# cloneofsimo/paint-with-words-sd

Measured on AMD Instinct MI355X. Metric: 512x512 images/sec (30 steps, CFG) SD1.5+PwW, higher is better.
Workload: dtype bf16

## Files before the change

include/pww_hip_linear.h:

```cpp
#ifndef PWW_HIP_LINEAR_H
#define PWW_HIP_LINEAR_H

#include "pww_hip.h"

#ifdef __cplusplus
extern "C" {
#endif

#define PWW_LINEAR_VERSION 100

int pww_linear_version(void);
const char *pww_linear_last_error(void);

#define PWW_LINEAR_NONE 0
#define PWW_LINEAR_BIAS 1
#define PWW_LINEAR_BIAS_RESIDUAL 2
#define PWW_LINEAR_BIAS_GEGLU 3
typedef struct pww_linear_desc {
    uint32_t size;
    int32_t dtype;
    int32_t M, N, K;
    int32_t epilogue;
    int64_t x_stride, y_stride, r_stride;
    int32_t tile_n, splitk;
} pww_linear_desc_t;
size_t pww_linear_workspace_bytes(const pww_linear_desc_t *desc);
int pww_linear_fwd(const void *x, const void *w, const void *bias, const void *residual, void *y, const pww_linear_desc_t *desc, void *workspace,
                   size_t workspace_bytes, void *stream);

#ifdef __cplusplus
}
#endif

#endif
```

paint-with-words-sd_amd/build.py:

```python
import os
import subprocess
import sys

HERE = os.path.dirname(os.path.abspath(__file__))
REPO = os.path.dirname(HERE)
CSRC = os.path.join(HERE, "csrc")
LIB = os.path.join(HERE, "pww_hip", "libpww_hip.so")
LIB_EXPERIMENTS = os.path.join(HERE, "pww_hip", "libpww_hip_experiments.so")
UNITS = [("pww_api.hip", [], ""), ("pww_attn.hip", [], ""), ("pww_cross.hip", [], ""), ("pww_cross_lean.hip", [], ""), ("pww_reduce.hip", [], ""),
         ("pww_mask.hip", [], ""), ("pww_qproj.hip", [], ""), ("pww_norm.hip", [], ""), ("pww_blocks.hip", [], ""), ("pww_conv.hip", [], ""), ("pww_probs.hip", [], ""),
         ("pww_attn_inst.hip", ["-DPWW_INST_F16"], ".f16"), ("pww_attn_inst.hip", ["-DPWW_INST_BF16"], ".bf16"),
         ("pww_cross_inst.hip", ["-DPWW_INST_F16", "-DPWW_INST_NW=2"], ".f16.nw2"), ("pww_cross_inst.hip", ["-DPWW_INST_F16", "-DPWW_INST_NW=4"], ".f16.nw4"),
         ("pww_cross_inst.hip", ["-DPWW_INST_BF16", "-DPWW_INST_NW=2"], ".bf16.nw2"), ("pww_cross_inst.hip", ["-DPWW_INST_BF16", "-DPWW_INST_NW=4"], ".bf16.nw4")]
EXPERIMENT_UNITS = [("pww_cross_out.hip", [], "")]
_ATTN_HEADERS = ["pww_tile.h", "pww_attn_core.h", "pww_cross_tile.h"]
SIDE_FLAGS = ["-fvisibility=hidden"]
SIDE_LIBS = {
    "long": ("pww_long.hip", _ATTN_HEADERS, "the long-prompt launches"),
    "scope": ("pww_scope.hip", _ATTN_HEADERS, "cross-attention with per-head / per-row score statistics"),
    "linear": ("pww_linear.hip", [], "linear layers with a bias / residual / GEGLU epilogue"),
    "regions": ("pww_regions.hip", [], "region masks and the per-pixel blend of the noise predictions"),
    "lora": ("pww_lora.hip", [], "the per-row low-rank update of unmerged LoRA adapters"),
}
SOURCES = sorted({u[0] for u in UNITS + EXPERIMENT_UNITS})
HEADERS = ["pww_common.h", "pww_tile.h", "pww_attn_core.h", "pww_attn_kernel.h", "pww_cross_tile.h", "pww_cross_kernel.h", os.path.join(REPO, "include", "pww_hip.h")]
SIDE_PATHS = {n: os.path.join(HERE, "pww_hip", "libpww_hip_%s.so" % n) for n in SIDE_LIBS}
SIDE_UNITS = {n: [(v[0], SIDE_FLAGS, "")] for n, v in SIDE_LIBS.items()}
LIB_LONG, LIB_SCOPE, LIB_LINEAR, LIB_REGIONS, LIB_LORA = (SIDE_PATHS[n] for n in ("long", "scope", "linear", "regions", "lora"))
LONG_UNITS, SCOPE_UNITS, LINEAR_UNITS, REGIONS_UNITS, LORA_UNITS = (SIDE_UNITS[n] for n in ("long", "scope", "linear", "regions", "lora"))
HIPCC = os.environ.get("HIPCC", "/opt/rocm/bin/hipcc")
FLAGS = ["--offload-arch=gfx950", "-O3", "-std=c++17", "-fPIC", "-Wall",
         "-Wno-unused-function", "-mllvm", "-amdgpu-kernarg-preload-count=16"]


PER_FILE_FLAGS = {"pww_mask.hip": ["-ffp-contract=off"], "pww_regions.hip": ["-ffp-contract=off"]}


def _newer(target, deps):
    if not os.path.exists(target):
        return True
    t = os.path.getmtime(target)
    return any(os.path.getmtime(d) > t for d in deps)


def _deps():
    return ([os.path.join(CSRC, s) for s in SOURCES] + [h if os.path.isabs(h) else os.path.join(CSRC, h) for h in HEADERS] + [__file__])


def _build(lib, units, defines, objdir, verbose, jobs=None):
    os.makedirs(objdir, exist_ok=True)
    order = sorted(units, key=lambda u: {"pww_cross_inst.hip": 0, "pww_attn_inst.hip": 1, "pww_cross_lean.hip": 2}.get(u[0], 3))
    jobs = jobs or max(2, min(len(order), os.cpu_count() or 4, int(os.environ.get("MAX_JOBS", 16))))
    pending, running, objs = list(order), [], []
# ... 77 lines not shown
```

paint-with-words-sd_amd/csrc/pww_linear.hip:

```cpp
#define PWW_SIDE_LIB "libpww_hip_linear"
#include "pww_side_host.h"
#include "../../include/pww_hip_linear.h"

#define PWW_LINEAR_API extern "C" __attribute__((visibility("default")))

namespace pww {

namespace {

constexpr int LN_BM = 128, LN_THREADS = 256;
constexpr int LN_PF = 2;

__device__ __forceinline__ f32x4 mfma16(f16x8 a, f16x8 b, f32x4 c) { return __builtin_amdgcn_mfma_f32_16x16x32_f16(a, b, c, 0, 0, 0); }
__device__ __forceinline__ f32x4 mfma16(bf16x8 a, bf16x8 b, f32x4 c) { return __builtin_amdgcn_mfma_f32_16x16x32_bf16(a, b, c, 0, 0, 0); }

struct LinCold {
    const void *bias, *residual;
    long ys, rs;
    int nsplit, nslab, mode, inner;
};

__device__ __forceinline__ int xcd_remap(int orig, int nwg) {
    const int xcd = orig & 7, q = nwg >> 3, r = nwg & 7;
    return (xcd < r ? xcd * (q + 1) : r * (q + 1) + (xcd - r) * q) + (orig >> 3);
}

template <typename T> __device__ __forceinline__ float rnd(float v) { return (float)(T)v; }

template <typename T>
__device__ __forceinline__ void epilogue4(const f32x4 &a, const LinCold &cold, T *y, int m, int n) {
    typedef typename Vec<T>::v4 V4;
    V4 o;
#pragma unroll
    for (int j = 0; j < 4; ++j) o[j] = (T)a[j];
    if (cold.mode >= PWW_LINEAR_BIAS) {
        const V4 b = *reinterpret_cast<const V4 *>(reinterpret_cast<const T *>(cold.bias) + n);
#pragma unroll
        for (int j = 0; j < 4; ++j) o[j] = (T)((float)o[j] + (float)b[j]);
    }
    if (cold.mode == PWW_LINEAR_BIAS_RESIDUAL) {
        const V4 r = *reinterpret_cast<const V4 *>(reinterpret_cast<const T *>(cold.residual) + (long)m * cold.rs + n);
#pragma unroll
        for (int j = 0; j < 4; ++j) o[j] = (T)((float)r[j] + (float)o[j]);
    }
    *reinterpret_cast<V4 *>(y + (long)m * cold.ys + n) = o;
}

template <typename T>
__device__ __forceinline__ void geglu4(const f32x4 &av, const f32x4 &ag, const LinCold &cold, T *y, int m, int j0) {
    typedef typename Vec<T>::v4 V4;
    const V4 bv = *reinterpret_cast<const V4 *>(reinterpret_cast<const T *>(cold.bias) + j0);
    const V4 bg = *reinterpret_cast<const V4 *>(reinterpret_cast<const T *>(cold.bias) + cold.inner + j0);
    V4 o;
#pragma unroll
    for (int j = 0; j < 4; ++j) {
        const float hv = rnd<T>(rnd<T>(av[j]) + (float)bv[j]);
        const float g = rnd<T>(rnd<T>(ag[j]) + (float)bg[j]);
        const float ge = rnd<T>(0.5f * g * (1.f + erff(g * 0.70710678118654752440f)));
        o[j] = (T)(hv * ge);
    }
    *reinterpret_cast<V4 *>(y + (long)m * cold.ys + j0) = o;
}

template <typename T, int BN>
__global__ void __launch_bounds__(LN_THREADS, 2) linear_kernel(const T *__restrict__ x, const T *__restrict__ w, void *out, int M, int N, int K, int xs,
                                                               const LinCold cold) {
    typedef typename Vec<T>::v8 V8;
    constexpr int BM = LN_BM, PF = LN_PF, XL = BM * 8 / LN_THREADS, WL = BN * 8 / LN_THREADS, RM = 4, RN = BN / 32;
    constexpr int XBYTES = BM * 128, STAGE = (BM + BN) * 128;
    __shared__ __attribute__((aligned(16))) char lds[2 * STAGE];

    const int tid = threadIdx.x, lane = tid & 63, wave = tid >> 6, wm = wave >> 1, wn = wave & 1;
    const int ntm = (M + BM - 1) / BM;
    const int bid = xcd_remap(blockIdx.x, gridDim.x);
    const bool split = cold.nsplit > 1;
    const bool geglu = cold.mode == PWW_LINEAR_BIAS_GEGLU;
    const int tile = bid / cold.nsplit, ks = bid - tile * cold.nsplit;
    const int tm = tile % ntm, tn = tile / ntm;
    const int s_begin = (int)((long)ks * cold.nslab / cold.nsplit), s_end = (int)((long)(ks + 1) * cold.nslab / cold.nsplit);

    const int c = tid & 7;
    unsigned xoff[XL], woff[WL];
#pragma unroll
    for (int i = 0; i < XL; ++i) {
        int m = tm * BM + (tid >> 3) + 32 * i;
        m = m < M ? m : M - 1;
        xoff[i] = (unsigned)(m * xs + c * 8);
    }
#pragma unroll
    for (int j = 0; j < WL; ++j) {
        const int t = (tid >> 3) + 32 * j;
        const int u = t % (BN / 2);
        const int row = geglu ? (u >= BN / 4 ? cold.inner : 0) + tn * (BN / 2) + (t / (BN / 2)) * (BN / 4) + u % (BN / 4) : tn * BN + t;
        woff[j] = (unsigned)(row * K + c * 8);
    }
    const int swz = ((c ^ ((tid >> 3) & 7)) << 4);

    u32x4 xr[PF][XL], wr[PF][WL];
    const T *xnext = x + s_begin * 64, *wnext = w + s_begin * 64;
    auto load = [&](int p) {
#pragma unroll
        for (int i = 0; i < XL; ++i) xr[p][i] = *reinterpret_cast<const u32x4 *>(xnext + xoff[i]);
#pragma unroll
        for (int j = 0; j < WL; ++j) wr[p][j] = *reinterpret_cast<const u32x4 *>(wnext + woff[j]);
        xnext += 64;
        wnext += 64;
    };
    auto store = [&](int p, int buf) {
        char *base = lds + buf * STAGE;
#pragma unroll
        for (int i = 0; i < XL; ++i) *reinterpret_cast<u32x4 *>(base + ((tid >> 3) + 32 * i) * 128 + swz) = xr[p][i];
// ... 69 lines not shown
                *reinterpret_cast<f32x4 *>(reinterpret_cast<float *>(out) + ((long)ks * M + m) * N + col) = acc[r][i];
            }
        } else if (geglu) {
#pragma unroll
            for (int r = 0; r < RN / 2; ++r)
                geglu4<T>(acc[r][i], acc[r + RN / 2][i], cold, reinterpret_cast<T *>(out), m, tn * (BN / 2) + wn * (BN / 4) + r * 16 + fq * 4);
        } else {
#pragma unroll
            for (int r = 0; r < RN; ++r) epilogue4<T>(acc[r][i], cold, reinterpret_cast<T *>(out), m, tn * BN + wn * (BN / 2) + r * 16 + fq * 4);
        }
    }
}

template <typename T>
__global__ void __launch_bounds__(256) linear_fold_kernel(const float *__restrict__ ws, T *y, long n4, int N, long MN, const LinCold cold) {
    const long q = (long)blockIdx.x * 256 + threadIdx.x;
    if (q >= n4) return;
    const bool geglu = cold.mode == PWW_LINEAR_BIAS_GEGLU;
    const int nout = geglu ? cold.inner : N;
    const long o4 = q * 4;
    const int m = (int)(o4 / nout), n = (int)(o4 - (long)m * nout);
    const float *p = ws + (long)m * N + n;
    f32x4 a = *reinterpret_cast<const f32x4 *>(p);
    for (int s = 1; s < cold.nsplit; ++s) a += *reinterpret_cast<const f32x4 *>(p + s * MN);
    if (geglu) {
        f32x4 g = *reinterpret_cast<const f32x4 *>(p + cold.inner);
        for (int s = 1; s < cold.nsplit; ++s) g += *reinterpret_cast<const f32x4 *>(p + s * MN + cold.inner);
        geglu4<T>(a, g, cold, y, m, n);
    } else {
        epilogue4<T>(a, cold, y, m, n);
    }
}

struct LinTune { int M, N, nslab, geglu, bn, nsplit; };
constexpr LinTune LIN_TUNED[] = {
    {8192, 2560, 5, 1, 64, 1}, {2048, 5120, 10, 1, 64, 1}, {512, 10240, 20, 1, 64, 1}, {128, 10240, 20, 1, 64, 1},
    {8192, 320, 20, 0, 64, 1}, {8192, 320, 5, 0, 64, 1}, {2048, 640, 40, 0, 128, 3}, {2048, 640, 10, 0, 64, 1},
    {512, 1280, 80, 0, 64, 3}, {512, 1280, 20, 0, 64, 2}, {128, 1280, 80, 0, 64, 5}, {128, 1280, 20, 0, 64, 4},
};

struct LinPlan {
    int bn, nsplit, nslab, ntiles, nout;
    long xs, ys, rs;
};

bool plan_linear(const pww_linear_desc_t *d, LinPlan *p) {
    if (!d || d->size < sizeof(pww_linear_desc_t)) { set_error("linear: descriptor missing or older than this library (size %u)", d ? d->size : 0u); return false; }
    const int e = d->epilogue;
    const bool geglu = e == PWW_LINEAR_BIAS_GEGLU;
    if ((d->dtype != PWW_DTYPE_F16 && d->dtype != PWW_DTYPE_BF16) || d->M < 1 || d->K < 64 || d->K % 64 != 0 || d->N < 64 || d->N % 64 != 0
        || e < PWW_LINEAR_NONE || e > PWW_LINEAR_BIAS_GEGLU || (geglu && d->N % 128 != 0)) {
        set_error("linear: unsupported (dtype %d M %d N %d K %d epilogue %d): K and N multiples of 64, GEGLU's inner = N / 2 a multiple of 64", d->dtype,
                  d->M, d->N, d->K, e);
        return false;
    }
    p->nout = geglu ? d->N / 2 : d->N;
    p->xs = d->x_stride ? d->x_stride : d->K;
    p->ys = d->y_stride ? d->y_stride : p->nout;
    p->rs = d->r_stride ? d->r_stride : p->nout;
    if (p->xs < d->K || p->ys < p->nout || p->rs < p->nout || ((p->xs | p->ys | p->rs) & 7)) {
        set_error("linear: row strides must cover their rows and be multiples of 8 elements (x %ld y %ld r %ld)", p->xs, p->ys, p->rs);
        return false;
    }
    if ((long)d->M * p->xs >= (1L << 31) || (long)d->N * d->K >= (1L << 31) || (long)d->M * d->N >= (1L << 31)) { set_error("linear: tensor of 2^31 elements or more"); return false; }
    p->nslab = d->K / 64;
    const LinTune *tuned = nullptr;
    for (const LinTune &t : LIN_TUNED)
        if (t.M == d->M && t.N == d->N && t.nslab == p->nslab && t.geglu == (int)geglu) tuned = &t;
    p->bn = d->tile_n ? d->tile_n : tuned ? tuned->bn : (d->N % 128 == 0 ? 128 : 64);
    if ((p->bn != 64 && p->bn != 128) || d->N % p->bn != 0) { set_error("linear: tile_n %d does not divide N %d", d->tile_n, d->N); return false; }
    p->ntiles = (d->M + LN_BM - 1) / LN_BM * (d->N / p->bn);
    int ns = d->splitk;
    if (ns <= 0 && tuned && p->bn == tuned->bn) ns = tuned->nsplit;
    if (ns <= 0) {
        ns = (480 + p->ntiles / 2) / p->ntiles;
        if (ns > p->nslab / 4) ns = p->nslab / 4;
        if (ns < 1) ns = 1;
    }
    if (ns > p->nslab || ns > 64) { set_error("linear: split %d exceeds the %d K-slabs (or 64)", ns, p->nslab); return false; }
    p->nsplit = ns;
    return true;
}

template <typename T>
int linear_launch(const LinPlan &p, const pww_linear_desc_t *d, const void *x, const void *w, const void *bias, const void *residual, void *y, void *ws,
                  hipStream_t stream) {
    LinCold cold{bias, residual, p.ys, p.rs, p.nsplit, p.nslab, d->epilogue, d->N / 2};
    const T *xt = static_cast<const T *>(x), *wt = static_cast<const T *>(w);
    const dim3 grid(p.ntiles * p.nsplit), block(LN_THREADS);
    void *out = p.nsplit == 1 ? y : ws;
    if (p.bn == 128) launch_timed(linear_kernel<T, 128>, grid, block, 0, stream, xt, wt, out, d->M, d->N, d->K, (int)p.xs, cold);
    else launch_timed(linear_kernel<T, 64>, grid, block, 0, stream, xt, wt, out, d->M, d->N, d->K, (int)p.xs, cold);
    if (p.nsplit == 1) return check_hip(hipGetLastError(), "linear launch");
    const long MN = (long)d->M * d->N, n4 = (long)d->M * p.nout / 4;
    launch_timed(linear_fold_kernel<T>, dim3((unsigned)((n4 + 255) / 256)), dim3(256), 0, stream, static_cast<const float *>(ws), static_cast<T *>(y), n4,
                 d->N, MN, cold);
    return check_hip(hipGetLastError(), "linear fold launch");
}

bool al16(const void *a) { return (reinterpret_cast<uintptr_t>(a) & 15) == 0; }

}

size_t linear_workspace_bytes(const pww_linear_desc_t *d) {
    LinPlan p;
    if (!plan_linear(d, &p)) return 0;
    return p.nsplit > 1 ? (size_t)p.nsplit * d->M * d->N * sizeof(float) : 0;
}

int linear_fwd(const void *x, const void *w, const void *bias, const void *residual, void *y, const pww_linear_desc_t *d, void *workspace,
               size_t workspace_bytes, hipStream_t stream) {
    LinPlan p;
    if (!plan_linear(d, &p)) return PWW_ENOTSUP;
    if (!x || !w || !y) { set_error("linear: x, w and y are required"); return PWW_EINVAL; }
    if ((d->epilogue >= PWW_LINEAR_BIAS && !bias) || (d->epilogue == PWW_LINEAR_BIAS_RESIDUAL && !residual)) {
        set_error("linear: epilogue %d needs its bias%s", d->epilogue, d->epilogue == PWW_LINEAR_BIAS_RESIDUAL ? " and residual" : "");
        return PWW_EINVAL;
    }
    if (!al16(x) || !al16(w) || !al16(y) || (reinterpret_cast<uintptr_t>(bias) & 7) || (reinterpret_cast<uintptr_t>(residual) & 7)) {
        set_error("linear: x, w, y must be 16-byte aligned, bias and residual 8-byte aligned");
        return PWW_EINVAL;
    }
    const size_t need = p.nsplit > 1 ? (size_t)p.nsplit * d->M * d->N * sizeof(float) : 0;
    if (need && (!workspace || !al16(workspace) || workspace_bytes < need)) {
        set_error("linear: split %d needs a 16-byte aligned workspace of %zu bytes (got %zu)", p.nsplit, need, workspace_bytes);
        return PWW_EINVAL;
    }
    if (!arch_ok()) return PWW_ENOTSUP;
    if (d->dtype == PWW_DTYPE_F16) return linear_launch<f16>(p, d, x, w, bias, residual, y, workspace, stream);
    return linear_launch<bf16>(p, d, x, w, bias, residual, y, workspace, stream);
}

}

PWW_LINEAR_API int pww_linear_version(void) { return PWW_LINEAR_VERSION; }
PWW_LINEAR_API const char *pww_linear_last_error(void) { return pww::last_error(); }
PWW_LINEAR_API size_t pww_linear_workspace_bytes(const pww_linear_desc_t *desc) { return pww::linear_workspace_bytes(desc); }
PWW_LINEAR_API int pww_linear_fwd(const void *x, const void *w, const void *bias, const void *residual, void *y, const pww_linear_desc_t *desc,
                                  void *workspace, size_t workspace_bytes, void *stream) {
    return pww::linear_fwd(x, w, bias, residual, y, desc, workspace, workspace_bytes, static_cast<hipStream_t>(stream));
}
```

paint-with-words-sd_amd/pww_hip/_lib.py:

```python
import ctypes
import os

_HERE = os.path.dirname(os.path.abspath(__file__))
LIB_PATH = os.environ.get("PWW_HIP_LIB", os.path.join(_HERE, "libpww_hip.so"))
EXPERIMENTS_LIB_PATH = os.environ.get("PWW_HIP_EXPERIMENTS_LIB", os.path.join(_HERE, "libpww_hip_experiments.so"))

LONG_LIB_PATH = os.environ.get("PWW_HIP_LONG_LIB", os.path.join(_HERE, "libpww_hip_long.so"))
SCOPE_LIB_PATH = os.environ.get("PWW_HIP_SCOPE_LIB", os.path.join(_HERE, "libpww_hip_scope.so"))
LINEAR_LIB_PATH = os.environ.get("PWW_HIP_LINEAR_LIB", os.path.join(_HERE, "libpww_hip_linear.so"))
REGIONS_LIB_PATH = os.environ.get("PWW_HIP_REGIONS_LIB", os.path.join(_HERE, "libpww_hip_regions.so"))
LORA_LIB_PATH = os.environ.get("PWW_HIP_LORA_LIB", os.path.join(_HERE, "libpww_hip_lora.so"))

PWW_OK, PWW_EINVAL, PWW_ENOTSUP, PWW_EHIP = 0, -22, -95, -5
MIN_VERSION = 127
DTYPE_F16, DTYPE_BF16 = 0, 1
LAYOUT_NCHW, LAYOUT_NHWC = 0, 1
ACT_NONE, ACT_SILU = 0, 1
LINEAR_NONE, LINEAR_BIAS, LINEAR_BIAS_RESIDUAL, LINEAR_BIAS_GEGLU = 0, 1, 2, 3
MAX_HEAD_DIM = 160

EXPORTS = ("pww_version", "pww_has_experiments", "pww_last_error", "pww_device_arch", "pww_self_attn_fwd", "pww_cross_attn_fwd",
           "pww_cross_attn_fwd_stat", "pww_cross_attn_fwd_stat_ex",
           "pww_qk_reduce", "pww_mask_build", "pww_mask_build_rgb", "pww_mask_build_f32", "pww_resize_tokens", "pww_gauss_blur", "pww_inpaint_prep", "pww_cfg_combine", "pww_store_f32",
           "pww_workspace_bytes", "pww_profile_arm", "pww_profile_elapsed_us", "pww_profile_reset", "pww_debug_timeline", "pww_debug_path_counts",
           "pww_debug_last_attn_route",
           "pww_qproj_stat", "pww_qproj_parts", "pww_cross_attn_fwd_parts", "pww_mask_build_f32_levels", "pww_qk_parts", "pww_qk_parts_count",
           "pww_group_norm_fwd", "pww_group_norm_workspace_bytes", "pww_add_layer_norm", "pww_add_layer_norm_bias", "pww_geglu", "pww_bias_residual",
           "pww_conv3x3_workspace_bytes", "pww_conv3x3_fwd", "pww_cross_attn_probs")
EXPERIMENT_EXPORTS = ("pww_cross_attn_fwd_fused", "pww_cross_attn_fwd_fused_ex", "pww_cross_fused_workspace_bytes", "pww_cross_fused_state_bytes",
                      "pww_cross_attn_fwd_parts_out", "pww_cross_attn_out_supported")


LONG_EXPORTS = ("pww_long_version", "pww_long_last_error", "pww_long_qk_parts", "pww_long_qk_parts_count", "pww_long_cross_attn_fwd_parts",
                "pww_long_cross_attn_probs", "pww_long_profile_arm", "pww_long_profile_elapsed_us")
LONG_MIN_VERSION = 100
LONG_MIN_KEYS, LONG_MAX_KEYS = 129, 256


SCOPE_EXPORTS = ("pww_scope_version", "pww_scope_last_error", "pww_scope_head_parts_count", "pww_scope_head_parts", "pww_scope_cross_attn_fwd")
SCOPE_MIN_VERSION = 100
SCOPE_HEAD, SCOPE_ROW = 1, 2


LINEAR_EXPORTS = ("pww_linear_version", "pww_linear_last_error", "pww_linear_workspace_bytes", "pww_linear_fwd")
LINEAR_MIN_VERSION = 100


REGIONS_EXPORTS = ("pww_regions_version", "pww_regions_last_error", "pww_regions_masks", "pww_regions_combine")
REGIONS_MIN_VERSION = 100
REGIONS_MAX, REGIONS_MAX_PLANE, REGIONS_MAX_FEATHER = 8, 9216, 8.0


LORA_EXPORTS = ("pww_lora_version", "pww_lora_last_error", "pww_lora_fwd")
LORA_MIN_VERSION = 100
LORA_MAX_ADAPTERS, LORA_MAX_RANK, LORA_MAX_SEGMENTS = 8, 128, 3


class AttnDesc(ctypes.Structure):
    _fields_ = [("dtype", ctypes.c_int32), ("B", ctypes.c_int32), ("H", ctypes.c_int32), ("N", ctypes.c_int32),
                ("M", ctypes.c_int32), ("D", ctypes.c_int32),
                ("q_stride", ctypes.c_int64 * 3), ("k_stride", ctypes.c_int64 * 3),
                ("v_stride", ctypes.c_int64 * 3), ("o_stride", ctypes.c_int64 * 3),
                ("scale", ctypes.c_float), ("bias_stride", ctypes.c_int64 * 4)]


class CrossOpts(ctypes.Structure):
    _fields_ = [("size", ctypes.c_uint32), ("bias_cols", ctypes.c_int32), ("coeff_scalar_dev", ctypes.c_void_p),
                ("bias_compact", ctypes.c_void_p), ("col_idx", ctypes.c_void_p), ("R", ctypes.c_int32), ("gated_images", ctypes.c_int32),
                ("compact_stride", ctypes.c_int64 * 2), ("col_idx_stride", ctypes.c_int64)]


class QprojDesc(ctypes.Structure):
    _fields_ = [("dtype", ctypes.c_int32), ("B", ctypes.c_int32), ("N", ctypes.c_int32), ("Cin", ctypes.c_int32), ("H", ctypes.c_int32),
                ("D", ctypes.c_int32), ("M", ctypes.c_int32), ("x_stride", ctypes.c_int64 * 2), ("q_stride", ctypes.c_int64 * 2),
                ("k_stride", ctypes.c_int64 * 2)]


# ... 154 lines not shown
    if _exp is not None:
        return _exp
    if has_experiments():
        _exp = load()
        return _exp
    if not os.path.isfile(EXPERIMENTS_LIB_PATH):
        raise PwwHipError("libpww_hip_experiments.so not found at %s: this entry point is not part of the product library. Build it with "
                          "`python paint-with-words-sd_amd/build.py --experiments` (tests: the `experiments_lib` fixture does)." % EXPERIMENTS_LIB_PATH)
    lib = ctypes.CDLL(EXPERIMENTS_LIB_PATH)
    lib.pww_has_experiments.restype = ctypes.c_int
    if not lib.pww_has_experiments():
        raise PwwHipError("%s was not built with -DPWW_EXPERIMENTS=1" % EXPERIMENTS_LIB_PATH)
    _exp = _bind(lib, True)
    return _exp


_P = ctypes.POINTER
_vp, _i32, _i64, _f32, _f64, _sz, _int = ctypes.c_void_p, ctypes.c_int32, ctypes.c_int64, ctypes.c_float, ctypes.c_double, ctypes.c_size_t, ctypes.c_int
_HINT = "(rebuild: python paint-with-words-sd_amd/build.py, or __graft_entry__.build())"
SIDE = {
    "long": dict(path="LONG_LIB_PATH", exports=LONG_EXPORTS, min_version=LONG_MIN_VERSION, missing_ok=False, needs="prompts longer than 77 tokens need it", sigs={
        "pww_long_qk_parts": ([_vp, _vp, _vp, _P(AttnDesc), _i32, _i32, _vp, _sz, _vp], _int),
        "pww_long_qk_parts_count": ([_P(AttnDesc)], _i32),
        "pww_long_cross_attn_fwd_parts": ([_vp, _vp, _vp, _vp, _vp, _i32, _f32, _vp, _P(AttnDesc), _vp, _i32, _vp, _P(CrossOpts), _vp], _int),
        "pww_long_cross_attn_probs": ([_vp, _vp, _vp, _vp, _i32, _f64, _f32, _vp, _P(AttnDesc), _P(CrossOpts), _vp, _P(ProbsDesc), _vp], _int),
        "pww_long_profile_arm": ([], _int),
        "pww_long_profile_elapsed_us": ([_P(_f32)], _int)}),
    "scope": dict(path="SCOPE_LIB_PATH", exports=SCOPE_EXPORTS, min_version=SCOPE_MIN_VERSION, missing_ok=True, needs="per-head / per-row score statistics need it", sigs={
        "pww_scope_head_parts_count": ([_P(AttnDesc)], _i32),
        "pww_scope_head_parts": ([_vp, _vp, _vp, _P(AttnDesc), _i32, _vp, _sz, _vp], _int),
        "pww_scope_cross_attn_fwd": ([_vp, _vp, _vp, _vp, _vp, _i32, _i32, _f32, _vp, _P(AttnDesc), _vp, _i32, _vp, _P(CrossOpts), _vp], _int)}),
    "linear": dict(path="LINEAR_LIB_PATH", exports=LINEAR_EXPORTS, min_version=LINEAR_MIN_VERSION, missing_ok=False, needs="linear layers on the native kernel need it", sigs={
        "pww_linear_workspace_bytes": ([_P(LinearDesc)], _sz),
        "pww_linear_fwd": ([_vp, _vp, _vp, _vp, _vp, _P(LinearDesc), _vp, _sz, _vp], _int)}),
    "regions": dict(path="REGIONS_LIB_PATH", exports=REGIONS_EXPORTS, min_version=REGIONS_MIN_VERSION, missing_ok=False, needs="region prompts need it", sigs={
        "pww_regions_masks": ([_vp, _i32, _i32, _vp, _i32, _f32, _vp, _vp], _int),
        "pww_regions_combine": ([_vp, _vp, _vp, _vp, _f32, _vp, _i32, _i32, _i32, _i64, _i32, _vp], _int)}),
}
SIDE_MORE = {
    "lora": dict(path="LORA_LIB_PATH", exports=LORA_EXPORTS, min_version=LORA_MIN_VERSION, missing_ok=False, needs="LoRA adapters on the native kernel need it", sigs={
        "pww_lora_fwd": ([_vp, _vp, _vp, _vp, _vp, _vp, _P(LoraDesc), _vp], _int)}),
}
_side = {}


def side_spec(name):
    return SIDE[name] if name in SIDE else SIDE_MORE[name]


def load_side(name):
    lib = _side.get(name)
    if lib is not None:
        return lib
    spec = side_spec(name)
    path, so, pre = globals()[spec["path"]], "libpww_hip_%s.so" % name, "pww_%s_" % name
    if not os.path.isfile(path):
        if spec["missing_ok"]:
            return None
        raise PwwHipError("%s not found at %s: %s %s" % (so, path, spec["needs"], _HINT))
    try:
        lib = ctypes.CDLL(path)
        getattr(lib, pre + "version").restype = _int
        version = getattr(lib, pre + "version")()
    except (OSError, AttributeError) as e:
        raise PwwHipError("%s at %s cannot be loaded: %s %s" % (so, path, e, _HINT))
    if version // 100 != 1 or version < spec["min_version"]:
        raise PwwHipError("%s ABI version %d is not 1.x >= %d %s" % (so[:-3], version, spec["min_version"], _HINT))
# ... 62 lines not shown
```

paint-with-words-sd_amd/pww_hip/blocks.py:

```python
import os
import types
import warnings

import torch
import torch.nn as nn
import torch.nn.functional as F

from . import ops

FUSED_NORM = os.environ.get("PWW_FUSED_NORM", "1") != "0"
BATCHED_TEMB = os.environ.get("PWW_BATCHED_TEMB", "1") != "0"
FOLD_CONV_BIAS = os.environ.get("PWW_FOLD_CONV_BIAS", "1") != "0"
CONV1X1_AS_LINEAR = os.environ.get("PWW_CONV1X1_AS_LINEAR", "1") != "0"
LINEAR = os.environ.get("PWW_LINEAR", "1")
CONV3X3 = os.environ.get("PWW_CONV3X3", "1") != "0"


_STATS = {k: [0, 0] for k in ("group_norm", "resnet_block", "transformer_block", "geglu", "conv1x1", "conv3x3", "linear")}
_UNRATED = ("conv1x1", "conv3x3", "linear")
_warned = set()


def stats():
    out = {k: {"fused": v[0], "declined": v[1]} for k, v in _STATS.items()}
# ... 235 lines not shown
    n = ops.add_layer_norm(h, self.norm1.weight, self.norm1.bias, self.norm1.eps)
    h, n = ops.add_layer_norm(h, self.norm2.weight, self.norm2.bias, self.norm2.eps, a=self.attn1(n))
    h, n = ops.add_layer_norm(h, self.norm3.weight, self.norm3.bias, self.norm3.eps, a=self.attn2(n, context=context))
    lin = _ff_output_linear(self.ff) if LINEAR != "0" else None
    if lin is not None:
        g = self.ff.net[0](n)
        if _linear_route(g, lin.weight, lin.bias, "residual", residual=h):
            return ops.linear(g, lin.weight, lin.bias, residual=h)
        return lin(g) + h
    return self.ff(n) + h


def _ff_output_linear(ff):
    net = getattr(ff, "net", None)
    if net is None or len(net) != 3 or type(ff).__name__ != "FeedForward" or "forward" in ff.__dict__:
        return None
    owner = next((c for c in type(ff).__mro__ if "forward" in c.__dict__), None)
    if owner is None or owner.__name__ != "FeedForward":
        return None
    act, drop, lin = net[0], net[1], net[2]
    if act.__class__.__name__ != "GEGLU" or not isinstance(drop, nn.Dropout) or (drop.training and drop.p > 0):
        return None
    if type(lin) is not nn.Linear or lin.bias is None or lin._forward_hooks or lin._forward_pre_hooks or "forward" in lin.__dict__ or ff._forward_hooks or ff._forward_pre_hooks:
        return None
    return lin


LINEAR_ROUTES = frozenset([
    (8192, 320, 2560, "geglu"),
    (2048, 640, 5120, "geglu"),
    (512, 1280, 10240, "geglu"),
    (128, 1280, 10240, "geglu"),
    (512, 5120, 1280, "residual"),
])


def _linear_route(x, weight, bias, epilogue, residual=None):
    ok = (LINEAR != "0" and FUSED_NORM and not torch.is_autocast_enabled() and torch.is_tensor(x) and bias is not None and bias.dtype == x.dtype
          and not (torch.is_grad_enabled() and (x.requires_grad or weight.requires_grad)) and ops.linear_takes(x, weight, epilogue == "geglu", bias=bias, residual=residual)
          and (LINEAR == "force" or (x.numel() // x.shape[-1], x.shape[-1], weight.shape[0], epilogue) in LINEAR_ROUTES))
    _STATS["linear"][0 if ok else 1] += 1
    return ok


def _plain_linear(lin):
    return type(lin) is nn.Linear and lin.bias is not None and not lin._forward_hooks and not lin._forward_pre_hooks and "forward" not in lin.__dict__


def _geglu_forward(self, x, *args, **kwargs):
    if args or kwargs:
        _count("geglu", False, x, "arguments beyond (hidden_states): %s" % (sorted(kwargs) or len(args)))
        return self._pww_orig_forward(x, *args, **kwargs)
    if _plain_linear(self.proj) and _linear_route(x, self.proj.weight, self.proj.bias, "geglu"):
        _count("geglu", True)
        return ops.linear(x, self.proj.weight, self.proj.bias, geglu=True)
    h = self.proj(x)
    if FUSED_NORM and h.is_cuda and h.dtype in (torch.float16, torch.bfloat16) and h.shape[-1] % 16 == 0 and not torch.is_autocast_enabled() \
            and not (torch.is_grad_enabled() and h.requires_grad):
        _count("geglu", True)
        return ops.geglu(h)
    _count("geglu", False, h, _why_not(h))
    a, gate = h.chunk(2, dim=-1)
    return a * F.gelu(gate)


def install_blocks(unet):
    n_res = n_gn = 0
    owned = set()
    plans = {}
    for m in unet.modules():
        if m.__class__.__name__ == "ResnetBlock2D" and _resnet_covered(m):
            if "_pww_orig_forward" not in m.__dict__:
                m.__dict__["_pww_orig_forward"] = m.forward
                m.forward = types.MethodType(_resnet_forward, m)
                lin = getattr(m, "time_emb_proj", None)
                if BATCHED_TEMB and isinstance(lin, nn.Linear):
                    m.__dict__["_pww_temb_slot"] = plans.setdefault(lin.in_features, TembProjections()).register(m)
            owned.update((id(m.norm1), id(m.norm2), id(m.conv1), id(m.conv2)))
            n_res += 1
    for m in unet.modules():
        name, fwd = m.__class__.__name__, None
        if isinstance(m, nn.GroupNorm) and id(m) not in owned:
            fwd = _group_norm_forward
            n_gn += 1
        elif name == "BasicTransformerBlock" and _transformer_block_covered(m):
            fwd = _transformer_block_forward
        elif name == "GEGLU" and isinstance(getattr(m, "proj", None), nn.Linear):
            fwd = _geglu_forward
        elif _is_conv1x1(m):
            fwd = _conv1x1_forward
        elif name == "Upsample2D" and _upsample_conv(m) is not None:
            fwd = _upsample_forward
            owned.add(id(_upsample_conv(m)))
        elif _is_conv3x3(m) and id(m) not in owned:
            fwd = _conv3x3_forward
        if fwd is not None and "_pww_orig_forward" not in m.__dict__:
            m.__dict__["_pww_orig_forward"] = m.forward
            m.forward = types.MethodType(fwd, m)
    return n_res, n_gn


def uninstall_blocks(unet):
    for m in unet.modules():
        if "_pww_orig_forward" in m.__dict__:
            del m.__dict__["_pww_orig_forward"]
            m.__dict__.pop("forward", None)
            m.__dict__.pop("_pww_temb_slot", None)
```

paint-with-words-sd_amd/pww_hip/ops.py:

```python
import ctypes

import torch

from . import _lib
from ._lib import AttnDesc, CrossOpts, ProbsDesc, QprojDesc, Region, PwwHipError

_DT = {torch.float16: _lib.DTYPE_F16, torch.bfloat16: _lib.DTYPE_BF16}


def _stream():
    return ctypes.c_void_p(torch.cuda.current_stream().cuda_stream)


def _ptr(t):
    return ctypes.c_void_p(t.data_ptr()) if t is not None else ctypes.c_void_p(0)


def _require_gpu(*tensors):
    for t in tensors:
        if t is not None and not t.is_cuda:
            raise PwwHipError("pww_hip ops need tensors on a HIP device (got %s); there is no CPU path" % t.device)


def _rows_ok(t):
# ... 936 lines not shown
    ws = torch.empty(nbytes // 4, dtype=torch.float32, device=x.device) if nbytes else None
    with torch.cuda.device(x.device):
        _lib.check(lib.pww_conv3x3_fwd(_ptr(x), _ptr(w), _ptr(bias), _ptr(residual), _ptr(y), ctypes.byref(d), _ptr(ws), nbytes, _stream()), "pww_conv3x3_fwd")
    return y


def _linear_weight(weight):
    if not torch.is_tensor(weight) or weight.dim() not in (2, 4) or (weight.dim() == 4 and tuple(weight.shape[2:]) != (1, 1)):
        return None
    w = weight.detach().reshape(weight.shape[0], weight.shape[1]) if weight.dim() == 4 else weight.detach()
    return w if w.is_contiguous() and w.data_ptr() == weight.data_ptr() and w.data_ptr() % 16 == 0 else None


def linear_takes(x, weight, geglu=False, bias=None, residual=None, out=None):
    if not (torch.is_tensor(x) and x.is_cuda and x.dtype in _DT and x.dim() >= 2 and torch.is_tensor(weight) and weight.dtype == x.dtype):
        return False
    w = _linear_weight(weight)
    if w is None or x.shape[-1] != w.shape[1] or x.numel() == 0 or _rows(x, "linear") is None:
        return False
    N, K = w.shape
    rows, _, xs = _rows(x, "linear")
    if not (K % 64 == 0 and N % (128 if geglu else 64) == 0 and rows * xs < 2 ** 31 and rows * N < 2 ** 31 and N * K < 2 ** 31):
        return False
    if bias is not None and not (torch.is_tensor(bias) and bias.is_cuda and bias.dtype == x.dtype and tuple(bias.shape) == (N,) and bias.is_contiguous()
                                 and bias.data_ptr() % 8 == 0):
        return False
    shape = tuple(x.shape[:-1]) + (N // 2 if geglu else N,)
    for t in (residual, out):
        if t is not None and not (torch.is_tensor(t) and t.is_cuda and t.dtype == x.dtype and tuple(t.shape) == shape and _rows(t, "linear") is not None):
            return False
    return True


def linear(x, weight, bias=None, residual=None, geglu=False, tile_n=0, splitk=0, out=None):
    _require_gpu(x, weight, bias, residual, out)
    if not linear_takes(x, weight, geglu):
        raise PwwHipError("linear: needs a float16/bfloat16 [..., K] x with one row pitch and a dense [N, K] weight of its dtype, K and N multiples of 64%s"
                          % (" (geglu: N / 2 a multiple of 64)" if geglu else ""))
    w = _linear_weight(weight)
    N, K = w.shape
    M, _, xs = _rows(x, "linear")
    nout = N // 2 if geglu else N
    if (geglu or residual is not None) and bias is None:
        raise PwwHipError("linear: the residual and GEGLU epilogues need the bias")
    if geglu and residual is not None:
        raise PwwHipError("linear: geglu and residual exclude each other")
    if bias is not None:
        if bias.dtype != x.dtype or tuple(bias.shape) != (N,):
            raise PwwHipError("linear: bias must be a %s [%d]" % (x.dtype, N))
        bias = bias.contiguous() if bias.data_ptr() % 8 == 0 else bias.clone(memory_format=torch.contiguous_format)
    shape = tuple(x.shape[:-1]) + (nout,)
    rs = 0
    if residual is not None:
        if tuple(residual.shape) != shape or residual.dtype != x.dtype:
            raise PwwHipError("linear: residual must be a %s %s" % (x.dtype, shape))
        r = _rows(residual, "linear")
        if r is None:
            residual = residual.contiguous()
            r = _rows(residual, "linear")
        rs = r[2]
    if out is None:
        out = torch.empty(shape, dtype=x.dtype, device=x.device)
    elif tuple(out.shape) != shape or out.dtype != x.dtype or _rows(out, "linear") is None:
        raise PwwHipError("linear: out must be a %s %s whose rows have one pitch" % (x.dtype, shape))
    ys = _rows(out, "linear")[2]
    epi = _lib.LINEAR_BIAS_GEGLU if geglu else _lib.LINEAR_BIAS_RESIDUAL if residual is not None else _lib.LINEAR_BIAS if bias is not None else _lib.LINEAR_NONE
    d = _lib.LinearDesc(ctypes.sizeof(_lib.LinearDesc), _DT[x.dtype], M, N, K, epi, xs, ys, rs, int(tile_n), int(splitk))
    lib = _lib.load_linear()
    nbytes = int(lib.pww_linear_workspace_bytes(ctypes.byref(d)))
    ws = torch.empty(nbytes // 4, dtype=torch.float32, device=x.device) if nbytes else None
    with torch.cuda.device(x.device):
        _lib.check(lib.pww_linear_fwd(_ptr(x), _ptr(w), _ptr(bias), _ptr(residual), _ptr(out), ctypes.byref(d), _ptr(ws), nbytes, _stream()), "pww_linear_fwd", lib)
    return out


def lora_update_torch(y, x, A, B, row_adapter, row_scale, n_seg):
    R, ns = y.shape[0], y.shape[-1] // n_seg
    ra, rs = row_adapter[:R].reshape(R, 1, 1), row_scale[:R].reshape(R, 1, 1)
    wide = torch.promote_types(y.dtype, torch.float32)
    for i in range(A.shape[0]):
        on = (ra == i) & (rs != 0)
        for g in range(n_seg):
            u = torch.matmul(torch.matmul(x, A[i, g].t()), B[i, g].t())
            seg = y[..., g * ns:(g + 1) * ns]
            seg.copy_(torch.where(on, (seg.to(wide) + rs.to(wide) * u.to(wide)).to(y.dtype), seg))
    return y


def lora_takes(y, x, A, B, n_seg):
    if not (torch.is_tensor(y) and y.is_cuda and y.dtype in _DT and y.dim() == 3 and x.dim() == 3 and x.dtype == y.dtype == A.dtype == B.dtype
            and x.is_cuda and A.is_cuda and B.is_cuda and A.is_contiguous() and B.is_contiguous() and A.dim() == 4 and B.dim() == 4):
        return False
    (R, T, N), K, (n, seg, rank, _) = y.shape, x.shape[-1], A.shape
    if not (tuple(x.shape[:2]) == (R, T) and seg == n_seg and 1 <= n_seg <= _lib.LORA_MAX_SEGMENTS and 1 <= n <= _lib.LORA_MAX_ADAPTERS and A.shape[3] == K
            and N % n_seg == 0 and tuple(B.shape) == (n, n_seg, N // n_seg, rank) and rank in (32, 64, 96, 128) and K % 32 == 0 and (N // n_seg) % 16 == 0
            and 1 <= R <= 65535 and T >= 1):
        return False
    for t, w in ((x, K), (y, N)):
        rs, ts = (T * t.stride(1) if R == 1 else t.stride(0)), t.stride(1)
        if t.stride(2) != 1 or ts < w or rs < T * ts or rs % 8 or ts % 8 or t.data_ptr() % 16 or R * rs >= 2 ** 31:
            return False
    return A.data_ptr() % 16 == 0 and B.data_ptr() % 16 == 0 and A.numel() < 2 ** 31 and B.numel() < 2 ** 31


def lora_update(y, x, layer_stack, state, n_seg):
# ... 24 lines not shown
```

Before: 5.145.

## Fuse transformer proj_out with residual and add banded XCD tile ordering for linear

Adds a banded tile order to the linear kernel so each XCD works on a contiguous band of M tiles sized to keep weights and X tiles in a cache budget, with a planner and an explicit order entry point. The 2048x640 split-K shape moves to bn=64 with the banded order. Transformer2DModel forward is replaced so the final 1x1 proj_out conv runs as a linear with a fused residual add, and two new residual shapes are routed to the native linear. This removes a separate conv and add pass over the spatial activations, at the cost of a fragile forward override that depends on the diffusers signature.

```diff
diff --git a/include/pww_hip_linear.h b/include/pww_hip_linear.h
--- a/include/pww_hip_linear.h
+++ b/include/pww_hip_linear.h
@@ -16,6 +16,9 @@
 #define PWW_LINEAR_BIAS 1
 #define PWW_LINEAR_BIAS_RESIDUAL 2
 #define PWW_LINEAR_BIAS_GEGLU 3
+#define PWW_LINEAR_ORDER_PLAN 0
+#define PWW_LINEAR_ORDER_COLUMN 1
+#define PWW_LINEAR_ORDER_BANDED 2
 typedef struct pww_linear_desc {
     uint32_t size;
     int32_t dtype;
@@ -27,6 +30,8 @@
 size_t pww_linear_workspace_bytes(const pww_linear_desc_t *desc);
 int pww_linear_fwd(const void *x, const void *w, const void *bias, const void *residual, void *y, const pww_linear_desc_t *desc, void *workspace,
                    size_t workspace_bytes, void *stream);
+int pww_linear_fwd_order(const void *x, const void *w, const void *bias, const void *residual, void *y, const pww_linear_desc_t *desc, void *workspace,
+                         size_t workspace_bytes, int order, int band_m, void *stream);
 
 #ifdef __cplusplus
 }
diff --git a/paint-with-words-sd_amd/build.py b/paint-with-words-sd_amd/build.py
--- a/paint-with-words-sd_amd/build.py
+++ b/paint-with-words-sd_amd/build.py
@@ -18,7 +18,7 @@
 SIDE_LIBS = {
     "long": ("pww_long.hip", _ATTN_HEADERS, "the long-prompt launches"),
     "scope": ("pww_scope.hip", _ATTN_HEADERS, "cross-attention with per-head / per-row score statistics"),
-    "linear": ("pww_linear.hip", [], "linear layers with a bias / residual / GEGLU epilogue"),
+    "linear": ("pww_linear.hip", ["pww_linear_order.h"], "linear layers with a bias / residual / GEGLU epilogue"),
     "regions": ("pww_regions.hip", [], "region masks and the per-pixel blend of the noise predictions"),
     "lora": ("pww_lora.hip", [], "the per-row low-rank update of unmerged LoRA adapters"),
 }
diff --git a/paint-with-words-sd_amd/csrc/pww_linear.hip b/paint-with-words-sd_amd/csrc/pww_linear.hip
--- a/paint-with-words-sd_amd/csrc/pww_linear.hip
+++ b/paint-with-words-sd_amd/csrc/pww_linear.hip
@@ -1,5 +1,6 @@
 #define PWW_SIDE_LIB "libpww_hip_linear"
 #include "pww_side_host.h"
+#include "pww_linear_order.h"
 #include "../../include/pww_hip_linear.h"
 
 #define PWW_LINEAR_API extern "C" __attribute__((visibility("default")))
@@ -18,12 +19,8 @@
     const void *bias, *residual;
     long ys, rs;
     int nsplit, nslab, mode, inner;
+    int band;
 };
-
-__device__ __forceinline__ int xcd_remap(int orig, int nwg) {
-    const int xcd = orig & 7, q = nwg >> 3, r = nwg & 7;
-    return (xcd < r ? xcd * (q + 1) : r * (q + 1) + (xcd - r) * q) + (orig >> 3);
-}
 
 template <typename T> __device__ __forceinline__ float rnd(float v) { return (float)(T)v; }
 
@@ -72,11 +69,11 @@
 
     const int tid = threadIdx.x, lane = tid & 63, wave = tid >> 6, wm = wave >> 1, wn = wave & 1;
     const int ntm = (M + BM - 1) / BM;
-    const int bid = xcd_remap(blockIdx.x, gridDim.x);
+    const LinTile order = lin_order_tile(blockIdx.x, gridDim.x, ntm, N / BN, cold.nsplit, cold.band);
+    if (order.tm < 0) return;
     const bool split = cold.nsplit > 1;
     const bool geglu = cold.mode == PWW_LINEAR_BIAS_GEGLU;
-    const int tile = bid / cold.nsplit, ks = bid - tile * cold.nsplit;
-    const int tm = tile % ntm, tn = tile / ntm;
+    const int tm = order.tm, tn = order.tn, ks = order.ks;
     const int s_begin = (int)((long)ks * cold.nslab / cold.nsplit), s_end = (int)((long)(ks + 1) * cold.nslab / cold.nsplit);
 
     const int c = tid & 7;
@@ -212,19 +209,30 @@
     }
 }
 
-struct LinTune { int M, N, nslab, geglu, bn, nsplit; };
+struct LinTune { int M, N, nslab, geglu, bn, nsplit, order; };
 constexpr LinTune LIN_TUNED[] = {
     {8192, 2560, 5, 1, 64, 1}, {2048, 5120, 10, 1, 64, 1}, {512, 10240, 20, 1, 64, 1}, {128, 10240, 20, 1, 64, 1},
-    {8192, 320, 20, 0, 64, 1}, {8192, 320, 5, 0, 64, 1}, {2048, 640, 40, 0, 128, 3}, {2048, 640, 10, 0, 64, 1},
+    {8192, 320, 20, 0, 64, 1}, {8192, 320, 5, 0, 64, 1}, {2048, 640, 40, 0, 64, 3, PWW_LINEAR_ORDER_BANDED}, {2048, 640, 10, 0, 64, 1},
     {512, 1280, 80, 0, 64, 3}, {512, 1280, 20, 0, 64, 2}, {128, 1280, 80, 0, 64, 5}, {128, 1280, 20, 0, 64, 4},
 };
 
 struct LinPlan {
     int bn, nsplit, nslab, ntiles, nout;
+    int band, grid;
     long xs, ys, rs;
 };
 
-bool plan_linear(const pww_linear_desc_t *d, LinPlan *p) {
+int plan_band(int ntm, int N, int K) {
+    const long budget = 3L << 20, wbytes = (long)N * K * 2, xtile = (long)LN_BM * K * 2;
+    if (wbytes + xtile > budget) return 0;
+    const long fit = (budget - wbytes) / xtile;
+    if (fit >= ntm) return 0;
+    const int nb = (int)((ntm + fit - 1) / fit + LIN_XCDS - 1) / LIN_XCDS * LIN_XCDS;
+    const int band = (ntm + nb - 1) / nb;
+    return band < ntm ? band : 0;
+}
+
+bool plan_linear(const pww_linear_desc_t *d, LinPlan *p, int ask_order = PWW_LINEAR_ORDER_PLAN, int ask_band = 0) {
     if (!d || d->size < sizeof(pww_linear_desc_t)) { set_error("linear: descriptor missing or older than this library (size %u)", d ? d->size : 0u); return false; }
     const int e = d->epilogue;
     const bool geglu = e == PWW_LINEAR_BIAS_GEGLU;
@@ -259,15 +267,28 @@
     }
     if (ns > p->nslab || ns > 64) { set_error("linear: split %d exceeds the %d K-slabs (or 64)", ns, p->nslab); return false; }
     p->nsplit = ns;
+    const int ntm = (d->M + LN_BM - 1) / LN_BM, ntn = d->N / p->bn;
+    if (ask_order < PWW_LINEAR_ORDER_PLAN || ask_order > PWW_LINEAR_ORDER_BANDED || ask_band < 0) {
+        set_error("linear: order %d (0 planned, 1 column, 2 banded) or band_m %d (0 planned) out of range", ask_order, ask_band);
+        return false;
+    }
+    const int named = ask_order ? ask_order : tuned && p->bn == tuned->bn ? tuned->order : 0;
+    int band = 0;
+    if (named != PWW_LINEAR_ORDER_COLUMN) {
+        band = ask_band ? ask_band : plan_band(ntm, d->N, d->K);
+        if (!band && named == PWW_LINEAR_ORDER_BANDED) band = (ntm + LIN_XCDS - 1) / LIN_XCDS;
+    }
+    p->band = band < ntm ? band : 0;
+    p->grid = lin_order_grid(ntm, ntn, ns, p->band);
     return true;
 }
 
 template <typename T>
 int linear_launch(const LinPlan &p, const pww_linear_desc_t *d, const void *x, const void *w, const void *bias, const void *residual, void *y, void *ws,
                   hipStream_t stream) {
-    LinCold cold{bias, residual, p.ys, p.rs, p.nsplit, p.nslab, d->epilogue, d->N / 2};
+    LinCold cold{bias, residual, p.ys, p.rs, p.nsplit, p.nslab, d->epilogue, d->N / 2, p.band};
     const T *xt = static_cast<const T *>(x), *wt = static_cast<const T *>(w);
-    const dim3 grid(p.ntiles * p.nsplit), block(LN_THREADS);
+    const dim3 grid(p.grid), block(LN_THREADS);
     void *out = p.nsplit == 1 ? y : ws;
     if (p.bn == 128) launch_timed(linear_kernel<T, 128>, grid, block, 0, stream, xt, wt, out, d->M, d->N, d->K, (int)p.xs, cold);
     else launch_timed(linear_kernel<T, 64>, grid, block, 0, stream, xt, wt, out, d->M, d->N, d->K, (int)p.xs, cold);
@@ -289,9 +310,9 @@
 }
 
 int linear_fwd(const void *x, const void *w, const void *bias, const void *residual, void *y, const pww_linear_desc_t *d, void *workspace,
-               size_t workspace_bytes, hipStream_t stream) {
+               size_t workspace_bytes, int order, int band_m, hipStream_t stream) {
     LinPlan p;
-    if (!plan_linear(d, &p)) return PWW_ENOTSUP;
+    if (!plan_linear(d, &p, order, band_m)) return PWW_ENOTSUP;
     if (!x || !w || !y) { set_error("linear: x, w and y are required"); return PWW_EINVAL; }
     if ((d->epilogue >= PWW_LINEAR_BIAS && !bias) || (d->epilogue == PWW_LINEAR_BIAS_RESIDUAL && !residual)) {
         set_error("linear: epilogue %d needs its bias%s", d->epilogue, d->epilogue == PWW_LINEAR_BIAS_RESIDUAL ? " and residual" : "");
@@ -318,5 +339,9 @@
 PWW_LINEAR_API size_t pww_linear_workspace_bytes(const pww_linear_desc_t *desc) { return pww::linear_workspace_bytes(desc); }
 PWW_LINEAR_API int pww_linear_fwd(const void *x, const void *w, const void *bias, const void *residual, void *y, const pww_linear_desc_t *desc,
                                   void *workspace, size_t workspace_bytes, void *stream) {
-    return pww::linear_fwd(x, w, bias, residual, y, desc, workspace, workspace_bytes, static_cast<hipStream_t>(stream));
-}
+    return pww::linear_fwd(x, w, bias, residual, y, desc, workspace, workspace_bytes, PWW_LINEAR_ORDER_PLAN, 0, static_cast<hipStream_t>(stream));
+}
+PWW_LINEAR_API int pww_linear_fwd_order(const void *x, const void *w, const void *bias, const void *residual, void *y, const pww_linear_desc_t *desc,
+                                        void *workspace, size_t workspace_bytes, int order, int band_m, void *stream) {
+    return pww::linear_fwd(x, w, bias, residual, y, desc, workspace, workspace_bytes, order, band_m, static_cast<hipStream_t>(stream));
+}
diff --git a/paint-with-words-sd_amd/csrc/pww_linear_order.h b/paint-with-words-sd_amd/csrc/pww_linear_order.h
--- /dev/null
+++ b/paint-with-words-sd_amd/csrc/pww_linear_order.h
@@ -0,0 +1,69 @@
+#ifndef PWW_LINEAR_ORDER_H
+#define PWW_LINEAR_ORDER_H
+
+#if defined(__HIPCC__)
+#define PWW_ORDER_FN __host__ __device__ __forceinline__
+#else
+#define PWW_ORDER_FN inline
+#endif
+
+namespace pww {
+
+constexpr int LIN_XCDS = 8;
+
+struct LinTile { int tm, tn, ks; };
+
+PWW_ORDER_FN int lin_xcd_remap(int orig, int nwg) {
+    const int xcd = orig & 7, q = nwg >> 3, r = nwg & 7;
+    return (xcd < r ? xcd * (q + 1) : r * (q + 1) + (xcd - r) * q) + (orig >> 3);
+}
+
+PWW_ORDER_FN int lin_order_grid(int ntm, int ntn, int nsplit, int band) {
+    const int exact = ntm * ntn * nsplit;
+    if (band <= 0 || band >= ntm) return exact;
+    const int nb = (ntm + band - 1) / band;
+    if (nb < LIN_XCDS) return exact;
+    const int full = band * ntn * nsplit, last = (ntm - (nb - 1) * band) * ntn * nsplit;
+    int grid = 0;
+    for (int x = 0; x < LIN_XCDS; ++x) {
+        const int count = (nb - x + LIN_XCDS - 1) / LIN_XCDS;
+        const int slots = (count - 1) * full + (((nb - 1) & 7) == x ? last : full);
+        const int upto = (slots - 1) * LIN_XCDS + x + 1;
+        grid = upto > grid ? upto : grid;
+    }
+    return grid;
+}
+
+PWW_ORDER_FN LinTile lin_order_tile(int blk, int nwg, int ntm, int ntn, int nsplit, int band) {
+    LinTile t;
+    if (band <= 0 || band >= ntm) {
+        const int bid = lin_xcd_remap(blk, nwg), tile = bid / nsplit;
+        t.ks = bid - tile * nsplit;
+        t.tm = tile % ntm;
+        t.tn = tile / ntm;
+        return t;
+    }
+    const int nb = (ntm + band - 1) / band;
+    int b, r;
+    if (nb < LIN_XCDS) {
+        const int bid = lin_xcd_remap(blk, nwg), per = band * ntn * nsplit;
+        b = bid / per;
+        r = bid - b * per;
+    } else {
+        const int slot = blk >> 3, full = band * ntn * nsplit, i = slot / full;
+        b = (blk & 7) + LIN_XCDS * i;
+        r = slot - i * full;
+        if (b >= nb) { t.tm = t.tn = t.ks = -1; return t; }
+    }
+    const int rest = ntm - b * band, bm = rest < band ? rest : band;
+    const int tile = r / nsplit, tn = tile / bm;
+    if (tn >= ntn) { t.tm = t.tn = t.ks = -1; return t; }
+    t.ks = r - tile * nsplit;
+    t.tm = b * band + (tile - tn * bm);
+    t.tn = tn;
+    return t;
+}
+
+}
+
+#endif
diff --git a/paint-with-words-sd_amd/pww_hip/_lib.py b/paint-with-words-sd_amd/pww_hip/_lib.py
--- a/paint-with-words-sd_amd/pww_hip/_lib.py
+++ b/paint-with-words-sd_amd/pww_hip/_lib.py
@@ -17,6 +17,7 @@
 LAYOUT_NCHW, LAYOUT_NHWC = 0, 1
 ACT_NONE, ACT_SILU = 0, 1
 LINEAR_NONE, LINEAR_BIAS, LINEAR_BIAS_RESIDUAL, LINEAR_BIAS_GEGLU = 0, 1, 2, 3
+LINEAR_ORDER_PLAN, LINEAR_ORDER_COLUMN, LINEAR_ORDER_BANDED = 0, 1, 2
 MAX_HEAD_DIM = 160
 
 EXPORTS = ("pww_version", "pww_has_experiments", "pww_last_error", "pww_device_arch", "pww_self_attn_fwd", "pww_cross_attn_fwd",
@@ -42,7 +43,7 @@
 SCOPE_HEAD, SCOPE_ROW = 1, 2
 
 
-LINEAR_EXPORTS = ("pww_linear_version", "pww_linear_last_error", "pww_linear_workspace_bytes", "pww_linear_fwd")
+LINEAR_EXPORTS = ("pww_linear_version", "pww_linear_last_error", "pww_linear_workspace_bytes", "pww_linear_fwd", "pww_linear_fwd_order")
 LINEAR_MIN_VERSION = 100
 
 
@@ -263,7 +264,8 @@
         "pww_scope_cross_attn_fwd": ([_vp, _vp, _vp, _vp, _vp, _i32, _i32, _f32, _vp, _P(AttnDesc), _vp, _i32, _vp, _P(CrossOpts), _vp], _int)}),
     "linear": dict(path="LINEAR_LIB_PATH", exports=LINEAR_EXPORTS, min_version=LINEAR_MIN_VERSION, missing_ok=False, needs="linear layers on the native kernel need it", sigs={
         "pww_linear_workspace_bytes": ([_P(LinearDesc)], _sz),
-        "pww_linear_fwd": ([_vp, _vp, _vp, _vp, _vp, _P(LinearDesc), _vp, _sz, _vp], _int)}),
+        "pww_linear_fwd": ([_vp, _vp, _vp, _vp, _vp, _P(LinearDesc), _vp, _sz, _vp], _int),
+        "pww_linear_fwd_order": ([_vp, _vp, _vp, _vp, _vp, _P(LinearDesc), _vp, _sz, _int, _int, _vp], _int)}),
     "regions": dict(path="REGIONS_LIB_PATH", exports=REGIONS_EXPORTS, min_version=REGIONS_MIN_VERSION, missing_ok=False, needs="region prompts need it", sigs={
         "pww_regions_masks": ([_vp, _i32, _i32, _vp, _i32, _f32, _vp, _vp], _int),
         "pww_regions_combine": ([_vp, _vp, _vp, _vp, _f32, _vp, _i32, _i32, _i32, _i64, _i32, _vp], _int)}),
diff --git a/paint-with-words-sd_amd/pww_hip/blocks.py b/paint-with-words-sd_amd/pww_hip/blocks.py
--- a/paint-with-words-sd_amd/pww_hip/blocks.py
+++ b/paint-with-words-sd_amd/pww_hip/blocks.py
@@ -291,6 +291,8 @@
     (512, 1280, 10240, "geglu"),
     (128, 1280, 10240, "geglu"),
     (512, 5120, 1280, "residual"),
+    (8192, 320, 320, "residual"),
+    (2048, 640, 640, "residual"),
 ])
 
 
@@ -300,6 +302,56 @@
           and (LINEAR == "force" or (x.numel() // x.shape[-1], x.shape[-1], weight.shape[0], epilogue) in LINEAR_ROUTES))
     _STATS["linear"][0 if ok else 1] += 1
     return ok
+
+
+_T2D_PARAMS = (("hidden_states", "encoder_hidden_states"), ("hidden_states", "encoder_hidden_states", "timestep", "return_dict"))
+
+
+def _transformer2d_covered(m):
+    import inspect
+    if (not isinstance(getattr(m, "norm", None), nn.GroupNorm) or getattr(m, "use_linear_projection", False) or not getattr(m, "is_input_continuous", True)
+            or not _is_conv1x1(getattr(m, "proj_in", None)) or not _is_conv1x1(getattr(m, "proj_out", None)) or not isinstance(getattr(m, "transformer_blocks", None), nn.ModuleList)
+            or "forward" in m.__dict__ or type(m).__name__ != "Transformer2DModel"):
+        return False
+    try:
+        params = tuple(inspect.signature(type(m).forward).parameters)[1:]
+    except (TypeError, ValueError):
+        return False
+    if params not in _T2D_PARAMS:
+        return False
+    return "return_dict" not in params or "Transformer2DModelOutput" in getattr(type(m).forward, "__globals__", {})
+
+
+def _transformer2d_forward(self, *args, **kwargs):
+    params = self.__dict__["_pww_t2d_params"]
+    full = "return_dict" in params
+    conv = self.proj_out
+    call = dict(zip(params, args)) if len(args) <= len(params) and not set(params[:len(args)]) & set(kwargs) and set(kwargs) <= set(params) else None
+    if call is not None:
+        call.update(kwargs)
+    x = call.get("hidden_states") if call is not None else None
+    if (LINEAR == "0" or not FUSED_NORM or not CONV1X1_AS_LINEAR or not torch.is_tensor(x) or not x.is_cuda or x.dim() != 4 or x.dtype != conv.weight.dtype
+            or x.shape[2] * x.shape[3] <= 1 or not x.is_contiguous(memory_format=torch.channels_last) or torch.is_autocast_enabled()
+            or call.get("timestep") is not None
+            or conv._forward_hooks or conv._forward_pre_hooks or self._forward_hooks or self._forward_pre_hooks or "_pww_orig_forward" not in conv.__dict__):
+        return self._pww_orig_forward(*args, **kwargs)
+    context = call.get("encoder_hidden_states")
+    B, C, H, W = x.shape
+    h = self.proj_in(self.norm(x))
+    inner = h.shape[1]
+    h = h.permute(0, 2, 3, 1).reshape(B, H * W, inner)
+    for blk in self.transformer_blocks:
+        h = blk(h, context=context, timestep=None) if full else blk(h, context=context)
+    r = x.permute(0, 2, 3, 1).reshape(B * H * W, C)
+    if conv.out_channels == C and _linear_route(h.reshape(B * H * W, inner), conv.weight, conv.bias, "residual", residual=r):
+        out = ops.linear(h.reshape(B * H * W, inner), conv.weight, conv.bias, residual=r).view(B, H, W, C).permute(0, 3, 1, 2)
+    else:
+        out = conv(h.reshape(B, H, W, inner).permute(0, 3, 1, 2)) + x
+    if not full:
+        return out
+    if not call.get("return_dict", True):
+        return (out,)
+    return type(self).forward.__globals__["Transformer2DModelOutput"](sample=out)
 
 
 def _plain_linear(lin):
@@ -346,6 +398,10 @@
             fwd = _transformer_block_forward
         elif name == "GEGLU" and isinstance(getattr(m, "proj", None), nn.Linear):
             fwd = _geglu_forward
+        elif name == "Transformer2DModel" and _transformer2d_covered(m):
+            import inspect
+            fwd = _transformer2d_forward
+            m.__dict__["_pww_t2d_params"] = tuple(inspect.signature(type(m).forward).parameters)[1:]
         elif _is_conv1x1(m):
             fwd = _conv1x1_forward
         elif name == "Upsample2D" and _upsample_conv(m) is not None:
@@ -365,3 +421,4 @@
             del m.__dict__["_pww_orig_forward"]
             m.__dict__.pop("forward", None)
             m.__dict__.pop("_pww_temb_slot", None)
+            m.__dict__.pop("_pww_t2d_params", None)
diff --git a/paint-with-words-sd_amd/pww_hip/ops.py b/paint-with-words-sd_amd/pww_hip/ops.py
--- a/paint-with-words-sd_amd/pww_hip/ops.py
+++ b/paint-with-words-sd_amd/pww_hip/ops.py
@@ -992,7 +992,7 @@
     return True
 
 
-def linear(x, weight, bias=None, residual=None, geglu=False, tile_n=0, splitk=0, out=None):
+def linear(x, weight, bias=None, residual=None, geglu=False, tile_n=0, splitk=0, out=None, order=0, band_m=0):
     _require_gpu(x, weight, bias, residual, out)
     if not linear_takes(x, weight, geglu):
         raise PwwHipError("linear: needs a float16/bfloat16 [..., K] x with one row pitch and a dense [N, K] weight of its dtype, K and N multiples of 64%s"
@@ -1030,7 +1030,11 @@
     nbytes = int(lib.pww_linear_workspace_bytes(ctypes.byref(d)))
     ws = torch.empty(nbytes // 4, dtype=torch.float32, device=x.device) if nbytes else None
     with torch.cuda.device(x.device):
-        _lib.check(lib.pww_linear_fwd(_ptr(x), _ptr(w), _ptr(bias), _ptr(residual), _ptr(out), ctypes.byref(d), _ptr(ws), nbytes, _stream()), "pww_linear_fwd", lib)
+        if order or band_m:
+            _lib.check(lib.pww_linear_fwd_order(_ptr(x), _ptr(w), _ptr(bias), _ptr(residual), _ptr(out), ctypes.byref(d), _ptr(ws), nbytes, int(order), int(band_m),
+                                                _stream()), "pww_linear_fwd_order", lib)
+        else:
+            _lib.check(lib.pww_linear_fwd(_ptr(x), _ptr(w), _ptr(bias), _ptr(residual), _ptr(out), ctypes.byref(d), _ptr(ws), nbytes, _stream()), "pww_linear_fwd", lib)
     return out
 
 
```

Result: no change. 5.150 (median of 3 runs) (+0.1%).
